# davidnabergoj/nfmc

Hardware: AMD Instinct MI355X
Metric: chain-steps/sec (n_chains x iters / s), jump_mala + RealNVP, d=64 (higher is better)
Workload: dtype f32

## Files before the change

nfmc_amd/csrc/flow_b_kernels.hip:

```cpp
#include "flow_b_mh.hpp"
#include "run_parts.hpp"

namespace nfmc {

template <int CPL, int LPC, int HP, int RR = 10>
__global__ void __launch_bounds__(kBlock, 1) flow_mh_b2_kernel(NfmcFlowMhArgs a, int64_t tiles) {
    extern __shared__ __attribute__((aligned(16))) float lds[];
    constexpr int CPW = kWave / LPC;
    const int lane = threadIdx.x & 63, wave = threadIdx.x >> 6;
    const int g = lane % LPC, cw = lane / LPC;
    const int d = a.flow.d;
    const int64_t n = a.n;
    using Flow = FlowB<CPL, LPC, HP, false, true>;
    Flow::Img::stage(lds, a.flow, kBlock);
    __syncthreads();
    Flow fl;
    fl.init(lds, a.flow, g);
    QuadraticPot<CPL, LPC, true> pot;
    pot.init(a.pot, g, d);
    const bool revl = (a.flow.n_coupling & 1) != 0;
    const float base_c = -0.5f * (float)d * kLog2Pi;

    float sx[CPL], sxx[CPL];
#pragma unroll
    for (int i = 0; i < CPL; ++i) sx[i] = sxx[i] = 0.f;
    uint32_t n_acc = 0, n_bad = 0;
    constexpr unsigned long long leaders = group_leaders(LPC);
    static_assert(LPC >= 8, "two-chain layouts: 8 .. 64 lanes per chain");

    for (int64_t tile = blockIdx.x; tile < tiles; tile += gridDim.x) {
        const int64_t ra = 2 * ((tile * kWavesPerBlock + wave) * CPW + cw), rb = ra + 1;
        const bool act_a = ra < n, act_b = rb < n;
        const uint32_t gca = (uint32_t)(a.rng.chain_offset + (uint64_t)ra), gcb = gca + 1u;
        float xa[CPL], xb[CPL];
        load_row<CPL, LPC, true>(a.x, ra, d, g, act_a, xa);
        load_row<CPL, LPC, true>(a.x, rb, d, g, act_b, xb);
        float u_a, u_b;
        {
            const auto ca = pot.prepare(xa, g, d);
            const auto cb = pot.prepare(xb, g, d);
            float pa = 0.f, pb = 0.f;
#pragma unroll
            for (int i = 0; i < CPL; ++i) {
                pa += pot.term(ca, i, xa[i]);
                pb += pot.term(cb, i, xb[i]);
            }
            u_a = group_allreduce<LPC>(pa);
            u_b = group_allreduce<LPC>(pb);
        }
        float f_a, f_b;
        if (a.logq_cached) {
            f_a = act_a ? a.logq[ra] : 0.f;
            f_b = act_b ? a.logq[rb] : 0.f;
        } else {
            float wa[CPL], wb[CPL];
#pragma unroll
            for (int i = 0; i < CPL; ++i) {
                wa[i] = xa[i];
                wb[i] = xb[i];
            }
            float pa, pb;
            fl.forward2(wa, wb, pa, pb);
#pragma unroll
            for (int i = 0; i < CPL; ++i) {
                pa = fmaf(-0.5f * wa[i], wa[i], pa);
                pb = fmaf(-0.5f * wb[i], wb[i], pb);
            }
            f_a = group_allreduce<LPC>(pa) + base_c;
            f_b = group_allreduce<LPC>(pb) + base_c;
        }
        for (int s = 0; s < a.n_steps; ++s) {
            float za[CPL], zb[CPL];
            draw_latent<CPL, LPC, true, RR>(za, nullptr, a.rng.seed, a.rng.step0 + (uint32_t)s, gca, ra, n, d, g, revl);
            draw_latent<CPL, LPC, true, RR>(zb, nullptr, a.rng.seed, a.rng.step0 + (uint32_t)s, gcb, rb, n, d, g, revl);
            float pa = 0.f, pb = 0.f;
#pragma unroll
            for (int i = 0; i < CPL; ++i) {
                pa = fmaf(-0.5f * za[i], za[i], pa);
                pb = fmaf(-0.5f * zb[i], zb[i], pb);
            }
            float la, lb;
            fl.inverse2(za, zb, la, lb);
            pa -= la;
            pb -= lb;
            const float f_pa = group_allreduce<LPC>(pa) + base_c, f_pb = group_allreduce<LPC>(pb) + base_c;
            float qa = 0.f, qb = 0.f;
            {
                const auto ca = pot.prepare(za, g, d);
                const auto cb = pot.prepare(zb, g, d);
#pragma unroll
                for (int i = 0; i < CPL; ++i) {
                    qa += pot.term(ca, i, za[i]);
                    qb += pot.term(cb, i, zb[i]);
                }
            }
            const float u_pa = group_allreduce<LPC>(qa), u_pb = group_allreduce<LPC>(qb);
            const float lra = (-u_pa) - (-u_a) + f_a - f_pa, lrb = (-u_pb) - (-u_b) + f_b - f_pb;
            bool acc_a = true, acc_b = true;
            if (a.adjusted) {
                const uint32_t step = a.rng.step0 + (uint32_t)s;
                const uint4 r0 = philox4x32<RR>(gca, step, 0u, kTagJump, (uint32_t)a.rng.seed, (uint32_t)(a.rng.seed >> 32));
                const uint4 r1 = philox4x32<RR>(gcb, step, 0u, kTagJump, (uint32_t)a.rng.seed, (uint32_t)(a.rng.seed >> 32));
                acc_a = fast_ln(u32_to_uniform(r0.x)) < lra;
                acc_b = fast_ln(u32_to_uniform(r1.x)) < lrb;
                n_bad += (uint32_t)__popcll(__ballot(act_a && !(fabsf(lra) <= 3.0e38f)) & leaders);
                n_bad += (uint32_t)__popcll(__ballot(act_b && !(fabsf(lrb) <= 3.0e38f)) & leaders);
            }
            acc_a = acc_a && act_a;
            acc_b = acc_b && act_b;
            const uint64_t ma = __ballot(acc_a), mb = __ballot(acc_b);
            n_acc += (uint32_t)__popcll(ma & leaders) + (uint32_t)__popcll(mb & leaders);
            f_a = select_f32(ma, f_pa, f_a);
            f_b = select_f32(mb, f_pb, f_b);
            u_a = select_f32(ma, u_pa, u_a);
            u_b = select_f32(mb, u_pb, u_b);
#pragma unroll
            for (int i = 0; i < CPL; ++i) {
                xa[i] = select_f32(ma, za[i], xa[i]);
                xb[i] = select_f32(mb, zb[i], xb[i]);
                sx[i] += xa[i];
                sxx[i] = fmaf(xa[i], xa[i], sxx[i]);
                sx[i] += xb[i];
                sxx[i] = fmaf(xb[i], xb[i], sxx[i]);
            }
        }
        store_row<CPL, LPC, true>(a.x, ra, d, g, act_a, xa);
        store_row<CPL, LPC, true>(a.x, rb, d, g, act_b, xb);
        if (g == 0 && act_a) a.logq[ra] = f_a;
        if (g == 0 && act_b) a.logq[rb] = f_b;
    }
    if (a.stats.sum_x) block_stats_flush<CPL, LPC>(sx, sxx, n_acc, n_bad, a.stats);
}

static bool wants_diag(const NfmcFlowMhArgs& a) {
    return a.rng.replay_normals || a.rng.replay_uniforms || a.samples.base || a.masks_out || a.log_ratio_out;
}

template <int CPL, int LPC, int HP>
static int launch_b2(const NfmcFlowMhArgs& a, int64_t tiles, int grid, hipStream_t st, bool dry) {
    if constexpr (CPL >= 8 && LPC >= 8) {
        const size_t lds = (size_t)FlowImage<CPL, LPC, HP, true>::total_floats(a.flow.n_hidden_layers, a.flow.n_coupling) * sizeof(float);
        if (lds > 120 * 1024) return NFMC_EUNSUPPORTED;
        if (dry) return 0;
        auto kern = rng_rounds(a.rng) == 7 ? flow_mh_b2_kernel<CPL, LPC, HP, 7> : flow_mh_b2_kernel<CPL, LPC, HP, 10>;
        return launch_lds(kern, grid, kBlock, lds, st, a, tiles);
    } else {
        return NFMC_EUNSUPPORTED;
    }
}

template <int CPL, int LPC, int HP>
static int launch_b_rqs(const NfmcFlowMhArgs& a, bool fast, int64_t tiles, int grid, hipStream_t st, bool dry) {
#define NFMC_LBR(POT, F)                                                                                          \
    {                                                                                                             \
        const size_t img = (size_t)FlowImage<CPL, LPC, HP, (F && CPL >= 8), kRqsBins>::total_floats(a.flow.n_hidden_layers, \
                                                                                                 a.flow.n_coupling) * sizeof(float); \
        const size_t lds = lds_with_potential(img, a.pot, CPL, LPC);                                             \
        if (lds > 120 * 1024) return NFMC_EUNSUPPORTED;                                                           \
        if (rng_rounds(a.rng) == 7) return NFMC_EUNSUPPORTED;                                                     \
        if (dry) return 0;                                                                                        \
        return launch_lds(flow_mh_b_kernel<CPL, LPC, HP, POT, F, true, 10, kRqsBins>, grid, kBlock, lds, st, a, tiles); \
    }
    if (a.pot.kind == NFMC_POT_GAUSSIAN_MIXTURE) NFMC_LBR(MixturePot, false)
    else if (a.pot.kind == NFMC_POT_LOGISTIC_REGRESSION) NFMC_LBR(LogRegPot, false)
    else if (a.pot.kind == NFMC_POT_FUNNEL) NFMC_LBR(FunnelPot, false)
    else if (fast) NFMC_LBR(QuadraticPot, true)
    else NFMC_LBR(QuadraticPot, false)
#undef NFMC_LBR
}

template <int CPL, int LPC, int HP>
static int launch_b(const NfmcFlowMhArgs& a, bool fast, int64_t tiles, int grid, hipStream_t st, bool dry) {
#define NFMC_LB(POT, F)                                                                                         \
    {                                                                                                           \
        const size_t img = (size_t)FlowImage<CPL, LPC, HP, (F && CPL >= 8)>::total_floats(a.flow.n_hidden_layers, \
                                                                                       a.flow.n_coupling) * sizeof(float); \
        const size_t lds = lds_with_potential(img, a.pot, CPL, LPC);                                           \
        if (lds > 120 * 1024) return NFMC_EUNSUPPORTED;                                                         \
        if (dry) return 0;                                                                                      \
        const bool diag = !F || wants_diag(a);                                                                  \
        const bool r7 = rng_rounds(a.rng) == 7;             \
        if (r7 && !F) return NFMC_EUNSUPPORTED;                                                                 \
        auto kern = r7 ? (diag ? flow_mh_b_kernel<CPL, LPC, HP, POT, F, true, (F ? 7 : 10)>                        \
                               : flow_mh_b_kernel<CPL, LPC, HP, POT, F, (F ? false : true), (F ? 7 : 10)>)         \
                       : (diag ? flow_mh_b_kernel<CPL, LPC, HP, POT, F, true>                                      \
                               : flow_mh_b_kernel<CPL, LPC, HP, POT, F, (F ? false : true)>);                      \
        return launch_lds(kern, grid, kBlock, lds, st, a, tiles);                                               \
    }
    if (a.pot.kind == NFMC_POT_GAUSSIAN_MIXTURE) NFMC_LB(MixturePot, false)
    else if (a.pot.kind == NFMC_POT_LOGISTIC_REGRESSION) NFMC_LB(LogRegPot, false)
    else if (a.pot.kind == NFMC_POT_FUNNEL) NFMC_LB(FunnelPot, false)
    else if (fast) NFMC_LB(QuadraticPot, true)
    else NFMC_LB(QuadraticPot, false)
#undef NFMC_LB
}

int flow_mh_b_launch(const NfmcFlowMhArgs& args, hipStream_t st, int* grid_out, int* dp_out, bool dry, const LaunchPart* part,
                     int64_t* tile_chains_out) {
    NfmcFlowMhArgs a = args;
    const int d = a.flow.d;
    const int hp = a.flow.n_hidden <= 4 ? 4 : 8;
    if (a.flow.n_hidden > 8 || d > 512) return NFMC_EUNSUPPORTED;
    BCfg c = {0, 0};
    const int want_cpl = (part ? part->layout_n : a.n) <= 4096 ? 4 : 8;
    for (const BCfg& k : kFlowBCfgs) {
        if (k.cpl * k.lpc < d) continue;
        if (c.cpl == 0 || k.cpl * k.lpc < c.cpl * c.lpc || (k.cpl * k.lpc == c.cpl * c.lpc && k.cpl == want_cpl)) c = k;
    }
    if (const char* e = getenv("NFMC_FLOWB_CFG")) {
        int cc = 0, ll = 0;
        if (sscanf(e, "%d,%d", &cc, &ll) == 2)
            for (const BCfg& k : kFlowBCfgs)
                if (k.cpl == cc && k.lpc == ll && cc * ll >= d) c = k;
    }
    if (!c.cpl) return NFMC_EUNSUPPORTED;
    const int dp = c.cpl * c.lpc;
    const bool fast = d == dp && (d % 4) == 0 && a.pot.a == nullptr && a.pot.b == nullptr &&
                      (((uintptr_t)a.x) & 15u) == 0 && (!a.samples.base || (((uintptr_t)a.samples.base) & 15u) == 0);
    const bool rqs = a.flow.n_bins != 0;
    if (rqs && (a.flow.n_bins != kRqsBins || !(a.flow.spline_bound > 0.f))) return NFMC_EUNSUPPORTED;
    bool dual = fast && c.cpl >= 8 && c.lpc >= 8 && a.pot.kind != NFMC_POT_FUNNEL && !wants_diag(a) && dp >= 256;
    if (const char* e = getenv("NFMC_FLOWB_DUAL"))
        dual = atoi(e) != 0 && fast && c.cpl >= 8 && c.lpc >= 8 && a.pot.kind != NFMC_POT_FUNNEL && !wants_diag(a);
    dual = dual && !rqs;
    const int cpw = (kWave / c.lpc) * (dual ? 2 : 1);
    const int64_t tiles = (a.n + (int64_t)kWavesPerBlock * cpw - 1) / ((int64_t)kWavesPerBlock * cpw);
    int gcap = dp <= 128 ? 1024 : 512;
    if (const char* e = getenv("NFMC_FLOWB_GRID")) gcap = atoi(e) > 0 ? atoi(e) : gcap;
    if (part && part->grid_cap < gcap) gcap = part->grid_cap;
    const int grid = (int)(tiles < gcap ? tiles : gcap);
    if (tile_chains_out) *tile_chains_out = (int64_t)kWavesPerBlock * cpw;
    if (a.stats.sum_x && a.stats.scratch_bytes < (int64_t)grid * (2 * dp + kStatTail) * (int64_t)sizeof(double))
        return NFMC_ESCRATCH;
    if (check_defer(a.stats, dp, d)) return NFMC_EINVAL;
    if (part && a.stats.sum_x) a.stats.scratch += (size_t)part->slab0 * (2 * dp + kStatTail);
    int rc = NFMC_EUNSUPPORTED;
    switch (a.pot.kind) {
#define NFMC_KIND_CASE(KIND, POT)                                                                    \
    case KIND:                                                                                       \
        rc = rqs ? launch_b_kind<POT, kRqsBins>(a, c, hp, tiles, grid, st, dry) : launch_b_kind<POT, 0>(a, c, hp, tiles, grid, st, dry); \
        break;
        NFMC_FOR_OWN_UNIT_POT(NFMC_KIND_CASE)
#undef NFMC_KIND_CASE
    default:
#define M(CPL, LPC)                                                                      \
    if (c.cpl == CPL && c.lpc == LPC)                                                    \
        rc = rqs ? (hp == 4 ? launch_b_rqs<CPL, LPC, 4>(a, fast, tiles, grid, st, dry) : launch_b_rqs<CPL, LPC, 8>(a, fast, tiles, grid, st, dry)) \
           : dual ? (hp == 4 ? launch_b2<CPL, LPC, 4>(a, tiles, grid, st, dry) : launch_b2<CPL, LPC, 8>(a, tiles, grid, st, dry)) \
                  : (hp == 4 ? launch_b<CPL, LPC, 4>(a, fast, tiles, grid, st, dry) : launch_b<CPL, LPC, 8>(a, fast, tiles, grid, st, dry));
        NFMC_FOR_FLOWB_CFG(M)
#undef M
    }
    *grid_out = grid;
    *dp_out = dp;
    return rc;
}

}
```

nfmc_amd/csrc/flow_b_mh.hpp:

```cpp
#pragma once

#include "flow_b.hpp"

namespace nfmc {

template <int CPL, int LPC, int HP, template <int, int, bool> class Pot, bool FAST, bool DIAG, int RR = 10, int NB = 0>
#ifndef NFMC_FLOWB_WPE
#define NFMC_FLOWB_WPE 1
#endif
__global__ void __launch_bounds__(kBlock, NFMC_FLOWB_WPE) flow_mh_b_kernel(NfmcFlowMhArgs a, int64_t tiles) {
    extern __shared__ __attribute__((aligned(16))) float lds[];
    constexpr int CPW = kWave / LPC;
    const int lane = threadIdx.x & 63, wave = threadIdx.x >> 6;
    const int g = lane % LPC, cw = lane / LPC;
    const int d = a.flow.d;
    const int64_t n = a.n;
    using Flow = FlowB<CPL, LPC, HP, false, (FAST && CPL >= 8), NB>;
    Flow::Img::stage(lds, a.flow, kBlock);
    __syncthreads();
    Flow fl;
    fl.init(lds, a.flow, g);
    Pot<CPL, LPC, FAST> pot;
    if constexpr (Pot<CPL, LPC, FAST>::kStaged)
        init_staged(pot, a.pot, g, d, lds, Flow::Img::total_floats(a.flow.n_hidden_layers, a.flow.n_coupling));
    else
        pot.init(a.pot, g, d);
    const bool revl = (a.flow.n_coupling & 1) != 0;
    const float base_c = -0.5f * (float)d * kLog2Pi;

    float sx[CPL], sxx[CPL];
#pragma unroll
    for (int i = 0; i < CPL; ++i) sx[i] = sxx[i] = 0.f;
    uint32_t n_acc = 0, n_bad = 0;
    constexpr unsigned long long leaders = group_leaders(LPC);

    for (int64_t tile = blockIdx.x; tile < tiles; tile += gridDim.x) {
        const int64_t row = (tile * kWavesPerBlock + wave) * CPW + cw;
        const bool active = row < n;
        const uint32_t gchain = (uint32_t)(a.rng.chain_offset + (uint64_t)row);
        float x[CPL];
        load_row<CPL, LPC, FAST>(a.x, row, d, g, active, x);
        float u_x;
        {
            const auto ctx = pot.prepare(x, g, d);
            float up = 0.f;
#pragma unroll
            for (int i = 0; i < CPL; ++i) up += pot.term(ctx, i, x[i]);
            u_x = group_allreduce<LPC>(up);
        }
        float f_x;
        if (a.logq_cached) {
            f_x = active ? a.logq[row] : 0.f;
        } else {
            float w[CPL];
#pragma unroll
            for (int i = 0; i < CPL; ++i) w[i] = x[i];
            float part = fl.forward(w);
#pragma unroll
            for (int i = 0; i < CPL; ++i) part = fmaf(-0.5f * w[i], w[i], part);
            f_x = group_allreduce<LPC>(part) + base_c;
        }
        StoreCursor keep(a.samples);
        for (int s = 0; s < a.n_steps; ++s) {
            float xp[CPL];
            draw_latent<CPL, LPC, FAST, RR>(xp, (DIAG && a.rng.replay_normals) ? a.rng.replay_normals + (int64_t)s * n * d : nullptr, a.rng.seed,
                                  a.rng.step0 + (uint32_t)s, gchain, row, n, d, g, revl);
            float part = 0.f;
#pragma unroll
            for (int i = 0; i < CPL; ++i) part = fmaf(-0.5f * xp[i], xp[i], part);
            part -= fl.inverse(xp);
            const float f_xp = group_allreduce<LPC>(part) + base_c;
            float up = 0.f;
            {
                const auto ctx = pot.prepare(xp, g, d);
#pragma unroll
                for (int i = 0; i < CPL; ++i) up += pot.term(ctx, i, xp[i]);
            }
            const float u_xp = group_allreduce<LPC>(up);
            const float lr = (-u_xp) - (-u_x) + f_x - f_xp;
            bool accept = true;
            if (a.adjusted) {
                float u;
                if (DIAG && a.rng.replay_uniforms) {
                    u = active ? a.rng.replay_uniforms[(int64_t)s * n + row] : 0.5f;
                } else {
                    const uint4 r = philox4x32<RR>(gchain, a.rng.step0 + (uint32_t)s, 0u, kTagJump, (uint32_t)a.rng.seed,
                                                  (uint32_t)(a.rng.seed >> 32));
                    u = u32_to_uniform(r.x);
                }
                accept = fast_ln(u) < lr;
                n_bad += (uint32_t)__popcll(__ballot(active && !(fabsf(lr) <= 3.0e38f)) & leaders);
            }
            accept = accept && active;
            const uint64_t am = __ballot(accept);
            n_acc += (uint32_t)__popcll(am & leaders);
            f_x = select_f32(am, f_xp, f_x);
            u_x = select_f32(am, u_xp, u_x);
#pragma unroll
            for (int i = 0; i < CPL; ++i) {
                x[i] = select_f32(am, xp[i], x[i]);
                sx[i] += x[i];
                sxx[i] = fmaf(x[i], x[i], sxx[i]);
            }
            if constexpr (DIAG) {
                if (float* kept = keep.next(n * d)) store_row<CPL, LPC, FAST>(kept, row, d, g, active, x);
            }
            if (DIAG && g == 0 && active) {
                if (a.masks_out) a.masks_out[(int64_t)s * n + row] = accept ? 1 : 0;
                if (a.log_ratio_out) a.log_ratio_out[(int64_t)s * n + row] = lr;
            }
        }
        store_row<CPL, LPC, FAST>(a.x, row, d, g, active, x);
        if (g == 0 && active) a.logq[row] = f_x;
    }
    if (a.stats.sum_x) block_stats_flush<CPL, LPC>(sx, sxx, n_acc, n_bad, a.stats);
}

struct BCfg {
    int cpl, lpc;
};
#define NFMC_FOR_FLOWB_CFG(M) M(4, 1) M(4, 2) M(4, 4) M(4, 8) M(8, 8) M(4, 16) M(8, 16) M(4, 32) M(8, 32) M(4, 64) M(8, 64)
#define NFMC_BCFG_ENTRY(CPL, LPC) {CPL, LPC},
constexpr BCfg kFlowBCfgs[] = {NFMC_FOR_FLOWB_CFG(NFMC_BCFG_ENTRY)};

template <template <int, int, bool> class POT, int NB>
int launch_b_kind(const NfmcFlowMhArgs& a, BCfg c, int hp, int64_t tiles, int grid, hipStream_t st, bool dry) {
    if (rng_rounds(a.rng) != 10) return NFMC_EUNSUPPORTED;
#define NFMC_AT(HP, CPL, LPC)                                                                                          \
    if (hp == HP && c.cpl == CPL && c.lpc == LPC) {                                                                    \
        const size_t img = (size_t)FlowImage<CPL, LPC, HP, false, NB>::total_floats(a.flow.n_hidden_layers, a.flow.n_coupling) * \
                           sizeof(float);                                                                              \
        const size_t lds = lds_with_potential(img, a.pot, CPL, LPC);                                                  \
        if (lds > 120 * 1024) return NFMC_EUNSUPPORTED;                                                                \
        return dry ? NFMC_OK : launch_lds(flow_mh_b_kernel<CPL, LPC, HP, POT, false, true, 10, NB>, grid, kBlock, lds, st, a, tiles); \
    }
#define M4(CPL, LPC) NFMC_AT(4, CPL, LPC)
#define M8(CPL, LPC) NFMC_AT(8, CPL, LPC)
    NFMC_FOR_FLOWB_CFG(M4) NFMC_FOR_FLOWB_CFG(M8)
#undef NFMC_AT
#undef M4
#undef M8
    return NFMC_EUNSUPPORTED;
}
#define NFMC_EXTERN_KIND(KIND, POT)                                                                                  \
    static_assert(kPotKinds[KIND].own_units, #POT);                                                                  \
    extern template int launch_b_kind<POT, 0>(const NfmcFlowMhArgs&, BCfg, int, int64_t, int, hipStream_t, bool);    \
    extern template int launch_b_kind<POT, kRqsBins>(const NfmcFlowMhArgs&, BCfg, int, int64_t, int, hipStream_t, bool);
NFMC_FOR_OWN_UNIT_POT(NFMC_EXTERN_KIND)
#undef NFMC_EXTERN_KIND

}
```

Baseline: 29.45 billion.

## Add lean high-occupancy flow MH kernel variant for quadratic potential

Adds a 'lean' dispatch path for the d=64 (8x8, hp=4) quadratic-potential configuration. It launches the flow MH kernel with a launch-bounds occupancy of 5 waves per EU, enables the FlowB lean-register template mode, raises wave priority with s_setprio, and uses asm barriers on lane indices to limit register rematerialisation. The aim is to hide latency through more resident waves, at the risk of register spills or LDS pressure. It is on by default only when a partition object is passed or when an env var forces it, and it falls back to the old path otherwise.

```diff
diff --git a/nfmc_amd/csrc/flow_b_kernels.hip b/nfmc_amd/csrc/flow_b_kernels.hip
--- a/nfmc_amd/csrc/flow_b_kernels.hip
+++ b/nfmc_amd/csrc/flow_b_kernels.hip
@@ -223,6 +223,9 @@
     if (const char* e = getenv("NFMC_FLOWB_DUAL"))
         dual = atoi(e) != 0 && fast && c.cpl >= 8 && c.lpc >= 8 && a.pot.kind != NFMC_POT_FUNNEL && !wants_diag(a);
     dual = dual && !rqs;
+    const char* lean_env = getenv("NFMC_FLOWB_LEAN");
+    const bool lean = (lean_env ? atoi(lean_env) != 0 : part != nullptr) && fast && !rqs && !dual &&
+                      a.pot.kind == NFMC_POT_QUADRATIC && lean_wpe(c, hp) > 0;
     const int cpw = (kWave / c.lpc) * (dual ? 2 : 1);
     const int64_t tiles = (a.n + (int64_t)kWavesPerBlock * cpw - 1) / ((int64_t)kWavesPerBlock * cpw);
     int gcap = dp <= 128 ? 1024 : 512;
@@ -243,6 +246,10 @@
         NFMC_FOR_OWN_UNIT_POT(NFMC_KIND_CASE)
 #undef NFMC_KIND_CASE
     default:
+        if (lean) {
+            rc = launch_b_lean(a, c, hp, wants_diag(a), tiles, grid, st, dry);
+            if (rc != NFMC_EUNSUPPORTED) break;
+        }
 #define M(CPL, LPC)                                                                      \
     if (c.cpl == CPL && c.lpc == LPC)                                                    \
         rc = rqs ? (hp == 4 ? launch_b_rqs<CPL, LPC, 4>(a, fast, tiles, grid, st, dry) : launch_b_rqs<CPL, LPC, 8>(a, fast, tiles, grid, st, dry)) \
diff --git a/nfmc_amd/csrc/flow_b_lean.hip b/nfmc_amd/csrc/flow_b_lean.hip
--- /dev/null
+++ b/nfmc_amd/csrc/flow_b_lean.hip
@@ -0,0 +1,35 @@
+#include "flow_b_mh.hpp"
+
+namespace nfmc {
+
+#define NFMC_FOR_LEAN_FORM(M) M(8, 8, 4, 5)
+
+int lean_wpe(BCfg c, int hp) {
+#define M(CPL, LPC, HP, WPE) \
+    if (c.cpl == CPL && c.lpc == LPC && hp == HP) return WPE;
+    NFMC_FOR_LEAN_FORM(M)
+#undef M
+    return 0;
+}
+
+int launch_b_lean(const NfmcFlowMhArgs& a, BCfg c, int hp, bool diag, int64_t tiles, int grid, hipStream_t st, bool dry) {
+    const bool r7 = rng_rounds(a.rng) == 7;
+#define M(CPL, LPC, HP, WPE)                                                                                           \
+    if (c.cpl == CPL && c.lpc == LPC && hp == HP) {                                                                    \
+        const size_t img = (size_t)FlowImage<CPL, LPC, HP, true>::total_floats(a.flow.n_hidden_layers, a.flow.n_coupling) * \
+                           sizeof(float);                                                                              \
+        const size_t lds = lds_with_potential(img, a.pot, CPL, LPC);                                                  \
+        if (lds > 120 * 1024) return NFMC_EUNSUPPORTED;                                                                \
+        if (dry) return NFMC_OK;                                                                                       \
+        auto kern = r7 ? (diag ? flow_mh_b_kernel<CPL, LPC, HP, QuadraticPot, true, true, 7, 0, WPE>                   \
+                               : flow_mh_b_kernel<CPL, LPC, HP, QuadraticPot, true, false, 7, 0, WPE>)                 \
+                       : (diag ? flow_mh_b_kernel<CPL, LPC, HP, QuadraticPot, true, true, 10, 0, WPE>                  \
+                               : flow_mh_b_kernel<CPL, LPC, HP, QuadraticPot, true, false, 10, 0, WPE>);               \
+        return launch_lds(kern, grid, kBlock, lds, st, a, tiles);                                                      \
+    }
+    NFMC_FOR_LEAN_FORM(M)
+#undef M
+    return NFMC_EUNSUPPORTED;
+}
+
+}
diff --git a/nfmc_amd/csrc/flow_b_mh.hpp b/nfmc_amd/csrc/flow_b_mh.hpp
--- a/nfmc_amd/csrc/flow_b_mh.hpp
+++ b/nfmc_amd/csrc/flow_b_mh.hpp
@@ -4,18 +4,23 @@
 
 namespace nfmc {
 
-template <int CPL, int LPC, int HP, template <int, int, bool> class Pot, bool FAST, bool DIAG, int RR = 10, int NB = 0>
 #ifndef NFMC_FLOWB_WPE
 #define NFMC_FLOWB_WPE 1
 #endif
-__global__ void __launch_bounds__(kBlock, NFMC_FLOWB_WPE) flow_mh_b_kernel(NfmcFlowMhArgs a, int64_t tiles) {
+#ifndef NFMC_FLOWB_LEAN_PRIO
+#define NFMC_FLOWB_LEAN_PRIO 3
+#endif
+template <int CPL, int LPC, int HP, template <int, int, bool> class Pot, bool FAST, bool DIAG, int RR = 10, int NB = 0,
+          int WPE = NFMC_FLOWB_WPE>
+__global__ void __launch_bounds__(kBlock, WPE) flow_mh_b_kernel(NfmcFlowMhArgs a, int64_t tiles) {
     extern __shared__ __attribute__((aligned(16))) float lds[];
     constexpr int CPW = kWave / LPC;
     const int lane = threadIdx.x & 63, wave = threadIdx.x >> 6;
     const int g = lane % LPC, cw = lane / LPC;
     const int d = a.flow.d;
     const int64_t n = a.n;
-    using Flow = FlowB<CPL, LPC, HP, false, (FAST && CPL >= 8), NB>;
+    if constexpr (WPE > 1) __builtin_amdgcn_s_setprio(NFMC_FLOWB_LEAN_PRIO);
+    using Flow = FlowB<CPL, LPC, HP, (WPE > 1), (FAST && CPL >= 8), NB>;
     Flow::Img::stage(lds, a.flow, kBlock);
     __syncthreads();
     Flow fl;
@@ -39,7 +44,9 @@
         const bool active = row < n;
         const uint32_t gchain = (uint32_t)(a.rng.chain_offset + (uint64_t)row);
         float x[CPL];
-        load_row<CPL, LPC, FAST>(a.x, row, d, g, active, x);
+        int gr = g;
+        if constexpr (WPE > 1) asm volatile("" : "+v"(gr));
+        load_row<CPL, LPC, FAST>(a.x, row, d, gr, active, x);
         float u_x;
         {
             const auto ctx = pot.prepare(x, g, d);
@@ -63,8 +70,10 @@
         StoreCursor keep(a.samples);
         for (int s = 0; s < a.n_steps; ++s) {
             float xp[CPL];
+            int gl = g;
+            if constexpr (WPE > 1) asm volatile("" : "+v"(gl));
             draw_latent<CPL, LPC, FAST, RR>(xp, (DIAG && a.rng.replay_normals) ? a.rng.replay_normals + (int64_t)s * n * d : nullptr, a.rng.seed,
-                                  a.rng.step0 + (uint32_t)s, gchain, row, n, d, g, revl);
+                                  a.rng.step0 + (uint32_t)s, gchain, row, n, d, gl, revl);
             float part = 0.f;
 #pragma unroll
             for (int i = 0; i < CPL; ++i) part = fmaf(-0.5f * xp[i], xp[i], part);
@@ -110,7 +119,9 @@
                 if (a.log_ratio_out) a.log_ratio_out[(int64_t)s * n + row] = lr;
             }
         }
-        store_row<CPL, LPC, FAST>(a.x, row, d, g, active, x);
+        int gs = g;
+        if constexpr (WPE > 1) asm volatile("" : "+v"(gs));
+        store_row<CPL, LPC, FAST>(a.x, row, d, gs, active, x);
         if (g == 0 && active) a.logq[row] = f_x;
     }
     if (a.stats.sum_x) block_stats_flush<CPL, LPC>(sx, sxx, n_acc, n_bad, a.stats);
@@ -122,6 +133,9 @@
 #define NFMC_FOR_FLOWB_CFG(M) M(4, 1) M(4, 2) M(4, 4) M(4, 8) M(8, 8) M(4, 16) M(8, 16) M(4, 32) M(8, 32) M(4, 64) M(8, 64)
 #define NFMC_BCFG_ENTRY(CPL, LPC) {CPL, LPC},
 constexpr BCfg kFlowBCfgs[] = {NFMC_FOR_FLOWB_CFG(NFMC_BCFG_ENTRY)};
+
+int lean_wpe(BCfg c, int hp);
+int launch_b_lean(const NfmcFlowMhArgs& a, BCfg c, int hp, bool diag, int64_t tiles, int grid, hipStream_t st, bool dry);
 
 template <template <int, int, bool> class POT, int NB>
 int launch_b_kind(const NfmcFlowMhArgs& a, BCfg c, int hp, int64_t tiles, int grid, hipStream_t st, bool dry) {
```

Result: faster. 30.32 billion, median of 6 (+2.9%).
